# lmwdhr/ViT-CNN

Hardware: AMD Instinct MI355X
Metric: training patches/sec, 9×9 HSI(144)+LiDAR patch, batch 64, 1/2/4/8 GPU (higher is better)
Workload: dtype fp32; 1 GPU; ViT-CNN (Multimodality_Mamba) train step, Houston2013 shape 144+1 bands, 9x9, 16 classes; global_batch=64, per_gpu_batch=64, parallelism=dp1, launch=hipGraph (whole step)

## Files before the change

include/vitcnn.h:

```cpp
#ifndef VITCNN_H
#define VITCNN_H

#include <stddef.h>
#include <hip/hip_runtime_api.h>

#ifdef __cplusplus
#define VC_API extern "C" __attribute__((visibility("default")))
#else
#define VC_API __attribute__((visibility("default")))
#endif

VC_API int vc_gemm(int transA, int transB, int M, int N, int K, float alpha,
                   const float* A, long lda, long strideA, const float* B, long ldb, long strideB,
                   float beta, float* C, long ldc, long strideC, int batch,
                   const float* bias, const float* addend, long add_ld, int add_mod, int flags,
                   float* bias_grad, float* ws, long ws_floats, hipStream_t stream);
VC_API int vc_gemm_ex(int transA, int transB, int M, int N, int K, float alpha, const float* A, long lda,
                      long strideA, const float* B, long ldb, long strideB, float beta, float* C, long ldc,
                      long strideC, int batch, const float* bias, const float* addend, long add_ld, int add_mod,
                      int flags, float* bias_grad, float* ws, long ws_floats, unsigned int* tile_counters,
                      int n_counters, hipStream_t stream);

VC_API int vc_gemm_tune(int bm, int bn, int nsplit, int pf, int combine);

// ... 92 lines not shown
                           float* col, float* ws, long ws_floats, hipStream_t stream);
VC_API int vc_col2im3x3(int B, int H, int W, int C, const float* dcol, float* dx, hipStream_t stream);

VC_API int vc_nonlocal_attn_pool_fwd(int B, int S, int P, int Ci, int Hs, const float* theta, const float* pg,
                                     long ldpg, float* pooled, unsigned char* arg, float* att, float* o,
                                     hipStream_t stream);
VC_API int vc_nonlocal_attn_pool_bwd(int B, int S, int P, int Ci, int Hs, const float* theta, const float* pooled,
                                     const float* att, const float* dout, const unsigned char* arg, float* dtheta,
                                     float* dpooled, float* dpg, hipStream_t stream);
VC_API int vc_maxpool2_fwd(int B, int H, int W, int C, const float* x, long ldx, float* y, unsigned char* arg,
                           hipStream_t stream);
VC_API int vc_maxpool2_bwd(int B, int H, int W, int C, const float* dy, const unsigned char* arg, float* dx,
                           long lddx, hipStream_t stream);

VC_API int vc_mamba_dirconv_fwd(int B, int L, int D, int ndir, const int* order, const float* xz,
                                const float* conv_w, const float* conv_b, float* u, hipStream_t stream);
VC_API int vc_mamba_scan_ckpt_floats(int B, int L, int D, int ndir);
VC_API int vc_mamba_scan_fwd(int B, int L, int D, int R, int ndir, const float* u, const float* xdbl,
                             const int* order, const float* dt_w, const float* dt_b, const float* A_log,
                             const float* Dskip, float* yp, float* ckpt, hipStream_t stream);
VC_API int vc_mamba_combine_fwd(int B, int L, int D, int ndir, const int* inv_order, const float* gate_logits,
                                const float* yp, const float* xz, float* ypsum, float* ysum, hipStream_t stream);
VC_API int vc_mamba_gate_bwd(int B, int L, int D, const float* xz, const float* ypsum, const float* dysum,
                             float* dyp, float* dxz, hipStream_t stream);
VC_API int vc_mamba_scan_bwd(int B, int L, int D, int R, int ndir, const float* u, const float* xdbl,
                             const int* order, const float* dt_w, const float* dt_b, const float* A_log,
                             const float* Dskip, const float* gate_logits, const float* yp, const float* dyp,
                             const float* ckpt, float* du, float* ddt_lin, float* dxdbl, float* dA_log,
                             float* dDskip, float* dgate_logits, float* ws, long ws_floats, hipStream_t stream);
VC_API int vc_mamba_scan_bwd_params(int B, int D, int ndir, const float* gate_logits, const float* ws,
                                    float* dA_log, float* dDskip, float* dgate_logits, float* scratch,
                                    long scratch_floats, hipStream_t stream);
VC_API int vc_mamba_dirconv_bwd(int B, int L, int D, int ndir, const int* order, const int* inv_order,
                                const float* xz, const float* conv_w, const float* conv_b, float* du, float* dxz,
                                float* dconv_w, float* dconv_b, float* ws, long ws_floats, hipStream_t stream);
VC_API int vc_mamba_scan_fwd_fused(int B, int L, int D, int R, int ndir, const float* xz, const int* order,
                                   const float* conv_w, const float* conv_b, const float* x_proj_w,
                                   const float* dt_w, const float* dt_b, const float* A_log, const float* Dskip,
                                   float* u, float* xdbl, float* yp, float* ckpt, hipStream_t stream);
VC_API int vc_mamba_scan_bwd_fused(int B, int L, int D, int R, int ndir, const float* u, const float* xdbl,
                                   const int* order, const float* xz, const float* conv_w, const float* conv_b,
                                   const float* x_proj_w, const float* dt_w, const float* dt_b, const float* A_log,
                                   const float* Dskip, const float* gate_logits, const float* yp, const float* dyp,
                                   const float* ckpt, float* dpre, float* ddt_lin, float* dxdbl, float* conv_part,
                                   float* dA_log, float* dDskip, float* dgate_logits, float* ws, long ws_floats,
                                   hipStream_t stream);
VC_API int vc_mamba_dirconv_bwd_gather(int B, int L, int D, int ndir, const int* inv_order, const float* conv_w,
                                       const float* dpre, float* dxz, hipStream_t stream);
VC_API int vc_mamba_conv_params(int B, int D, int ndir, const float* conv_part, float* dconv_w, float* dconv_b,
                                hipStream_t stream);
VC_API int vc_mamba_bwd_params(int B, int D, int ndir, const float* gate_logits, const float* ws, const float* conv_part,
                               float* dA_log, float* dDskip, float* dgate_logits, float* dconv_w, float* dconv_b,
                               hipStream_t stream);

VC_API int vc_rowchain_front(int rows, int K0, int E, int N2, const float* x, const float* w_embed, const float* pos,
                             int L, float* t, const float* ln_w, const float* ln_b, float eps, float* xn, float* mean,
                             float* rstd, const float* w_proj, float* out, hipStream_t stream);
VC_API int vc_rowchain_back(int B, int L, int D, int ndir, const int* inv_order, const float* gate_logits,
                            const float* yp, const float* xz, float* ypsum, float* ysum, int E, const float* w_out,
                            const float* residual, float* t2, const float* ln_w, const float* ln_b, float eps,
                            float* g, float* mean, float* rstd, int N2, const float* w_proj, const float* b_proj,
                            float* out, hipStream_t stream);

VC_API int vc_rowchain_back_bwd(int rows, int Cout, int E, int D, const float* dcd, const float* w_cd, const float* t2,
                                const float* mean, const float* rstd, const float* ln_w, float* dt, float* ln_part,
                                const float* w_out, const float* xz, const float* ypsum, float* dyp, float* dxz,
                                hipStream_t stream);
VC_API int vc_rowchain_front_bwd(int rows, int K0, int E, int Cin, const float* dxz, const float* w_in, const float* t,
                                 const float* mean, const float* rstd, const float* ln_w, const float* res, float* dtt,
                                 float* ln_part, const float* w_embed, float* dx, float beta, const float* dx_add,
                                 hipStream_t stream);
VC_API int vc_rowchain_ln_params(int rows, int E, const float* ln_part, float* dw, float* db, float beta,
                                 hipStream_t stream);
VC_API int vc_rowchain_ln_part_floats(int rows, int E);

VC_API int vc_tl_ws_floats(int B, int HW, int S);
VC_API int vc_tl_check(int HW, int C, int S);
VC_API int vc_tl_pixel_stats(long M, int C, const float* x, long ldx, float* mx, int* amx, float* avg, double* ws,
                             hipStream_t stream);
VC_API int vc_tl_fwd(int train, int B, int HW, int C, int S, const float* x, long ldx, const float* mx,
                     const float* avg, const float* params, float* bn_buffers, float eps, float momentum,
                     const double* ws, double* stats, float* a, float* Z, hipStream_t stream);
VC_API int vc_tl_bwd(int train, int B, int HW, int C, int S, const float* x, long ldx, const float* mx,
                     const float* avg, const int* amx, const float* params, const double* stats, const float* a,
                     const float* dZ, double* ws, float* dx, long lddx, float* dparams, hipStream_t stream);
VC_API int vc_tl_relu_mask(int B, int HW, int S, const float* mx, const float* avg, const float* params,
                           const double* stats, unsigned char* mask, hipStream_t stream);

VC_API int vc_nonlocal_attn_fwd(int B, int S, int P, int Ci, const float* theta, const float* pooled, float* att,
                                float* o, hipStream_t stream);
VC_API int vc_nonlocal_attn_bwd(int B, int S, int P, int Ci, const float* theta, const float* pooled,
                                const float* att, const float* dout, float* dtheta, float* dpooled,
                                hipStream_t stream);

VC_API int vc_cat2_fwd(long M, int C1, int C2, const float* x1, long ld1, const float* x2, long ld2, int exchange,
                       float* out, hipStream_t stream);
VC_API int vc_cat2_bwd(long M, int C1, int C2, const float* dout, int exchange, float* dx1, long ld1, float beta1,
                       float* dx2, long ld2, float beta2, hipStream_t stream);
VC_API int vc_glf_combine_fwd(long M, int C, const float* w_pre, const float* bn_mean, const float* bn_invstd,
                              const float* bn_w, const float* bn_b, const float* fc, const float* fl, float* out,
                              hipStream_t stream);
VC_API int vc_bn_glf_combine(long M, int C, const float* w_pre, float eps, float momentum, float* save_mean,
                             float* save_invstd, float* run_mean, float* run_var, const float* bn_w, const float* bn_b,
                             const float* fc, const float* fl, float* out, float* ws, long ws_floats,
                             hipStream_t stream);
VC_API int vc_add2_2d(long M, int C, const float* a, long lda, const float* b, long ldb, float* out, long ldo,
// ... 170 lines not shown
```

vit-cnn_amd/csrc/mamba.hip:

```cpp
#include "common.h"

namespace {

constexpr int NST = 16;

constexpr int DC_T = 8;
__global__ void dirconv_fwd_run(int total, FastDiv fD, FastDiv fC, FastDiv fB, int L, const int* __restrict__ order,
                                const float* __restrict__ xz, const float* __restrict__ cw,
                                const float* __restrict__ cb, float* __restrict__ u) {
  const int idx = blockIdx.x * blockDim.x + threadIdx.x;
  if (idx >= total) return;
  const int D = fD.div;
  int d, c, b;
  const int sc = fdivmod(idx, fD, d);
  const int sq = fdivmod(sc, fC, c);
  const int k = fdivmod(sq, fB, b);
  const int* ord = order + k * L;
  const float* xb = xz + (long)b * L * (2 * D) + d;
  const float w0 = cw[d * 4], w1 = cw[d * 4 + 1], w2 = cw[d * 4 + 2], w3 = cw[d * 4 + 3], bias = cb[d];
  const int t0 = c * DC_T;
  float x[DC_T + 3];
#pragma unroll
  for (int i = 0; i < DC_T + 3; ++i) {
    const int tau = t0 - 3 + i;
// ... 749 lines not shown
  const int b = fdivmod(bl, fL, l);
  float mx = logits[0];
  for (int i = 1; i < ndir; ++i) mx = fmaxf(mx, logits[i]);
  float den = 0.f;
  for (int i = 0; i < ndir; ++i) den += __expf(logits[i] - mx);
  const float rden = 1.f / den;
  float acc = 0.f;
  for (int k0 = 0; k0 < ndir; k0 += MAXK) {
    int tk[MAXK];
#pragma unroll
    for (int kk = 0; kk < MAXK; ++kk) tk[kk] = k0 + kk < ndir ? inv[(k0 + kk) * L + l] : 0;
    float yv[MAXK];
#pragma unroll
    for (int kk = 0; kk < MAXK; ++kk)
      yv[kk] = k0 + kk < ndir ? y[((long)((k0 + kk) * B + b) * L + tk[kk]) * D + d] : 0.f;
#pragma unroll
    for (int kk = 0; kk < MAXK; ++kk)
      if (k0 + kk < ndir) {
        const float gk = __expf(logits[k0 + kk] - mx) * rden;
        acc += gk * yv[kk];
      }
  }
  ypsum[idx] = acc;
  out[idx] = acc * silu_f(xz[(long)bl * 2 * D + D + d]);
}

__device__ __forceinline__ void gate_grad_body(int ndir, int per_dir, const float* __restrict__ logits,
                                               const float* __restrict__ part, float* __restrict__ dlogits,
                                               float* dg, float* gg) {
  const int lane = threadIdx.x & 63, wave = threadIdx.x >> 6;
  for (int kk = wave; kk < ndir; kk += 4) {
    float s = 0.f;
    for (int i = lane; i < per_dir; i += 64) s += part[(long)kk * per_dir + i];
    s = wave_sum(s);
    if (lane == 0) {
      dg[kk] = s;
      gg[kk] = gate_softmax(logits, ndir, kk);
    }
  }
  __syncthreads();
  if (threadIdx.x < ndir) {
    float dot = 0.f;
    for (int i = 0; i < ndir; ++i) dot += gg[i] * dg[i];
    dlogits[threadIdx.x] = gg[threadIdx.x] * (dg[threadIdx.x] - dot);
  }
}

__global__ __launch_bounds__(256) void gate_grad(int ndir, int per_dir, const float* __restrict__ logits,
                                                 const float* __restrict__ part, float* __restrict__ dlogits) {
  __shared__ float dg[64], gg[64];
  gate_grad_body(ndir, per_dir, logits, part, dlogits, dg, gg);
}

__global__ __launch_bounds__(256) void mamba_params(int nseq, int D, int ndir, int ncb, const float* __restrict__ logits,
                                                    const float* __restrict__ pa, const float* __restrict__ pd,
                                                    const float* __restrict__ pg, const float* __restrict__ cp,
                                                    float* __restrict__ dA, float* __restrict__ dDs,
                                                    float* __restrict__ dgl, float* __restrict__ dcw,
                                                    float* __restrict__ dcb) {
  __shared__ float sh[16][17];
  __shared__ float dg[64], gg[64];
  if ((int)blockIdx.x == ncb) {
    gate_grad_body(ndir, nseq / ndir, logits, pg, dgl, dg, gg);
    return;
  }
  const int cl = threadIdx.x & 15, pl = threadIdx.x >> 4;
  const int c = blockIdx.x * 16 + cl;
  const float* src = nullptr;
  long stride = 0;
  float* dst = nullptr;
  int cc = 0;
  if (c < NST * D) src = pa, stride = (long)NST * D, dst = dA, cc = c;
  else if (c < (NST + 1) * D) src = pd, stride = D, dst = dDs, cc = c - NST * D;
  else if (c < (NST + 5) * D) src = cp, stride = 5L * D, dst = dcw, cc = c - (NST + 1) * D;
  else if (c < (NST + 6) * D) src = cp + 4L * D, stride = 5L * D, dst = dcb, cc = c - (NST + 5) * D;
  float s = 0.f;
  if (src) {
#pragma unroll 4
    for (int p = pl; p < nseq; p += 16) s += src[(long)p * stride + cc];
  }
  sh[pl][cl] = s;
  __syncthreads();
  if (pl == 0 && src) {
    float v = 0.f;
#pragma unroll
    for (int i = 0; i < 16; ++i) v += sh[i][cl];
    dst[cc] = v;
  }
}


template <int MAXK>
__global__ void dirconv_bwd_gather(int total, FastDiv fD, FastDiv fL, int B, int ndir, const int* __restrict__ inv,
                                   const float* __restrict__ cw, const float* __restrict__ dpre,
                                   float* __restrict__ dxz) {
  const int idx = blockIdx.x * blockDim.x + threadIdx.x;
  if (idx >= total) return;
  const int D = fD.div, L = fL.div;
  int d, l;
  const int bl = fdivmod(idx, fD, d);
  const int b = fdivmod(bl, fL, l);
  float w[4];
#pragma unroll
  for (int j = 0; j < 4; ++j) w[j] = cw[d * 4 + j];
  float acc = 0.f;
  for (int k0 = 0; k0 < ndir; k0 += MAXK) {
    int tk[MAXK];
#pragma unroll
    for (int kk = 0; kk < MAXK; ++kk) tk[kk] = k0 + kk < ndir ? inv[(k0 + kk) * L + l] : L;
    float v[MAXK][4];
#pragma unroll
    for (int kk = 0; kk < MAXK; ++kk) {
      const float* base = dpre + (long)((k0 + kk) * B + b) * L * D + d;
#pragma unroll
      for (int j = 0; j < 4; ++j) {
        const int t = tk[kk] + 3 - j;
        v[kk][j] = t < L ? base[(long)t * D] : 0.f;
      }
    }
#pragma unroll
    for (int kk = 0; kk < MAXK; ++kk)
#pragma unroll
      for (int j = 0; j < 4; ++j) acc = fmaf(w[j], v[kk][j], acc);
  }
  dxz[(long)bl * 2 * D + d] = acc;
}

__global__ __launch_bounds__(256) void dirconv_bwd_wgrad(int D, int L, FastDiv fC, FastDiv fB,
                                                         const int* __restrict__ order, const float* __restrict__ xz,
                                                         const float* __restrict__ cw, const float* __restrict__ cb,
                                                         float* __restrict__ du, int items, int items_per,
                                                         float* __restrict__ part) {
  __shared__ float sh[5][16][17];
  const int dlc = threadIdx.x & 15, rl = threadIdx.x >> 4;
  const int d = blockIdx.x * 16 + dlc;
  const int i0 = blockIdx.y * items_per, i1 = min(items, i0 + items_per);
  float acc[5] = {0.f, 0.f, 0.f, 0.f, 0.f};
  if (d < D) {
    const float w0 = cw[d * 4], w1 = cw[d * 4 + 1], w2 = cw[d * 4 + 2], w3 = cw[d * 4 + 3], bias = cb[d];
    for (int it = i0 + rl; it < i1; it += 16) {
// ... 220 lines not shown
                                   float* u, float* xdbl, float* y, float* ckpt, hipStream_t stream) {
  VC_REQUIRE(B > 0 && L > 0 && D > 0 && D <= 128 && R > 0 && R <= 64 && ndir > 0);
  VC_REQUIRE(xz && order && conv_w && conv_b && x_proj_w && u && xdbl && scan_fusable(D, R));
  const dim3 grid(ndir * B), block(vc_cdiv(D, 16) * 64);
  VC_REQUIRE(block.x <= 512);
  const size_t sm = sizeof(float) * (seq_lds_floats(L, R, block.x / 4) + L);
  VC_REQUIRE(sm <= 160 * 1024);
  VC_REQUIRE_I32((long)ndir * B * L * (R + 2 * NST));
  VC_REQUIRE_I32((long)B * L * 2 * D);
  const ScanArgs a{B, L, D, R, u, xdbl, order, dt_w, dt_b, A_log, Dskip};
  const FusedFwd f{xz, conv_w, conv_b, x_proj_w, u, xdbl};
  if (R == 9) hipLaunchKernelGGL((scan_fwd<9, true>), grid, block, sm, stream, a, y, ckpt, f);
  else if (R == 16) hipLaunchKernelGGL((scan_fwd<16, true>), grid, block, sm, stream, a, y, ckpt, f);
  else hipLaunchKernelGGL((scan_fwd<0, true>), grid, block, sm, stream, a, y, ckpt, f);
  VC_CHECK_LAUNCH();
  return VC_OK;
}

VC_API int vc_mamba_dirconv_bwd_gather(int B, int L, int D, int ndir, const int* inv_order, const float* conv_w,
                                       const float* dpre, float* dxz, hipStream_t stream) {
  VC_REQUIRE(B > 0 && L > 0 && D > 0 && ndir > 0);
  VC_REQUIRE_I32((long)ndir * B * L * D);
  const long tot2 = (long)B * L * D;
  if (ndir <= 10)
    hipLaunchKernelGGL(dirconv_bwd_gather<10>, dim3(vc_cdiv(tot2, 256)), dim3(256), 0, stream, (int)tot2,
                       make_fastdiv(D), make_fastdiv(L), B, ndir, inv_order, conv_w, dpre, dxz);
  else
    hipLaunchKernelGGL(dirconv_bwd_gather<4>, dim3(vc_cdiv(tot2, 256)), dim3(256), 0, stream, (int)tot2,
                       make_fastdiv(D), make_fastdiv(L), B, ndir, inv_order, conv_w, dpre, dxz);
  VC_CHECK_LAUNCH();
  return VC_OK;
}

VC_API int vc_mamba_conv_params(int B, int D, int ndir, const float* conv_part, float* dconv_w, float* dconv_b,
                                hipStream_t stream) {
  VC_REQUIRE(B > 0 && D > 0 && ndir > 0 && conv_part && dconv_w && dconv_b);
  const int nseq = ndir * B;
  if (dconv_b == dconv_w + 4L * D) return launch_sum_rows(nseq, 5 * D, conv_part, 5L * D, 0L, dconv_w, 0.f, stream);
  const int rc = launch_sum_rows(nseq, 4 * D, conv_part, 5L * D, 0L, dconv_w, 0.f, stream);
  if (rc) return rc;
  return launch_sum_rows(nseq, D, conv_part, 5L * D, 4L * D, dconv_b, 0.f, stream);
}

VC_API int vc_mamba_bwd_params(int B, int D, int ndir, const float* gate_logits, const float* ws, const float* conv_part,
                               float* dA_log, float* dDskip, float* dgate_logits, float* dconv_w, float* dconv_b,
                               hipStream_t stream) {
  VC_REQUIRE(B > 0 && D > 0 && ndir > 0 && ndir <= 64 && gate_logits && ws && conv_part && dA_log && dDskip &&
             dgate_logits && dconv_w && dconv_b);
  const int nseq = ndir * B;
  const float* p_a = ws;
  const float* p_d = p_a + (long)nseq * D * NST;
  const float* p_g = p_d + (long)nseq * D;
  const int ncb = vc_cdiv((NST + 6) * D, 16);
  hipLaunchKernelGGL(mamba_params, dim3(ncb + 1), dim3(256), 0, stream, nseq, D, ndir, ncb, gate_logits, p_a, p_d,
                     p_g, conv_part, dA_log, dDskip, dgate_logits, dconv_w, dconv_b);
  VC_CHECK_LAUNCH();
  return VC_OK;
}

VC_API int vc_mamba_scan_bwd_params(int B, int D, int ndir, const float* gate_logits, const float* ws,
                                    float* dA_log, float* dDskip, float* dgate_logits, float* scratch,
                                    long scratch_floats, hipStream_t stream) {
  VC_REQUIRE(B > 0 && D > 0 && ndir > 0 && ws);
  const int nseq = ndir * B;
  const float* p_a = ws;
  const float* p_d = p_a + (long)nseq * D * NST;
  const float* p_g = p_d + (long)nseq * D;
  return scan_param_reduce(B, D, ndir, gate_logits, p_a, p_d, p_g, dA_log, dDskip, dgate_logits, scratch,
                           scratch_floats, stream);
}


VC_API int vc_mamba_dirconv_bwd(int B, int L, int D, int ndir, const int* order, const int* inv_order, const float* xz,
                                const float* conv_w, const float* conv_b, float* du, float* dxz,
                                float* dconv_w, float* dconv_b, float* ws, long ws_floats, hipStream_t stream) {
  VC_REQUIRE(B > 0 && L > 0 && D > 0 && ndir > 0);
  const long rows = (long)ndir * B * L;
  VC_REQUIRE_I32(rows * D);
  const int nch = vc_cdiv(L, DC_T);
  const long items = (long)ndir * B * nch;
  int items_per = std::max<long>(16, (items + 255) / 256);
  while ((long)vc_cdiv(items, items_per) * D * 5 > ws_floats) items_per *= 2;
  const int P = vc_cdiv(items, items_per);
  hipLaunchKernelGGL(dirconv_bwd_wgrad, dim3(vc_cdiv(D, 16), P), dim3(256), 0, stream, D, L, make_fastdiv(nch),
                     make_fastdiv(B), order, xz, conv_w, conv_b, du, (int)items, items_per, ws);
  VC_CHECK_LAUNCH();
  const long tot2 = (long)B * L * D;
  if (ndir <= 10)
    hipLaunchKernelGGL(dirconv_bwd_gather<10>, dim3(vc_cdiv(tot2, 256)), dim3(256), 0, stream, (int)tot2,
                       make_fastdiv(D), make_fastdiv(L), B, ndir, inv_order, conv_w, du, dxz);
  else
    hipLaunchKernelGGL(dirconv_bwd_gather<4>, dim3(vc_cdiv(tot2, 256)), dim3(256), 0, stream, (int)tot2,
                       make_fastdiv(D), make_fastdiv(L), B, ndir, inv_order, conv_w, du, dxz);
  VC_CHECK_LAUNCH();
  if (dconv_b == dconv_w + 4L * D) return launch_sum_rows(P, 5 * D, ws, 5L * D, 0L, dconv_w, 0.f, stream);
  int rc = launch_sum_rows(P, 4 * D, ws, 5L * D, 0L, dconv_w, 0.f, stream);
  if (rc) return rc;
  rc = launch_sum_rows(P, D, ws, 5L * D, 4L * D, dconv_b, 0.f, stream);
  if (rc) return rc;
  return VC_OK;
}
```

vit-cnn_amd/vitcnn_amd/model.py:

```python
from __future__ import annotations

import contextlib
import ctypes
import math
import sys
import weakref
from typing import Dict

import torch
import torch.nn as nn

from ._lib import lib
from .flat import install_grad_views
from .layers import ConvBnReluParams, FusionParams, GlobalLocalParams
from .scan_orders import scan_orders

F32 = 4
LN_EPS = 1e-6
BN_EPS = 1e-5
BN_MOM = 0.1
NDIR = 10
N_SIDE = 3
_ONE_PARAM_REDUCE = True
WGRAD_LANE = 2
WGRAD1_LANE = 3
_IMPLICIT_CONV = False
_DEFER_WGRAD = True
_DEFER_WGRAD1 = False
SIDE_SCRATCH = 1 << 23
PARAM_ALIGN = 4
ALIGN_MIN = 64
GEMM_GROUP_BYTES = 16384
GEMM_MASK = 64
_GLOBAL_FIRST = False
_GEMM_BNSTATS = True
_PG_LANE2 = False
N_COUNTERS = 1 << 16

_SCAN_FUSED = True
_ROW_CHAIN = True
_GLF_FUSED = True
_TAP_DGRAD = False
_LANES = True
_LANES_BWD = True
_TRACER = None
_GROUP = True
_BF16_EXACT: set = set()
_BF16_MIN_K = 0
_GEMM_SITES = None
_LANE_MAP = []
_CH_LANE = 1
_CH_ORDERED = True
_BN_RELU_AFFINE = True
_BN_TICKETS = False

UNUSED_PREFIXES = ("hsi1.global_view.tokenlearner.", "hsi1.global_view.ln3.",
                   "hsi2.global_view.tokenlearner.", "hsi2.global_view.ln3.")


PRECISIONS = ("fp32", "bf16")
GEMM_BF16 = 2


def _check_precision(p):
    if p not in PRECISIONS:
        raise ValueError(f"precision must be one of {PRECISIONS}, got {p!r}")
    return p


class _Workspace:

    def __init__(self, device):
        self.device = device
        self.t: Dict[str, torch.Tensor] = {}
        self.generation = 0

# ... 998 lines not shown
                if dX:
                    self.mm_nn(rows, Cin, Cout, dCF, Cout, self.P[pfx + ".channel_feature.weight"], Cin, dX, Cin,
                               beta=1.0)
            e_ch = (self.mark(), e_loc) if side else (self.mark(),)
            self.flush_wgrads1()
        Zg, dZg = f(pfx + ".global_feature.Z", M * Cout), f(pfx + ".dZg", M * Cout)
        self.ln_bwd(pfx + ".ln3", pfx + ".Fg", dFg, Zg, M, Cout, dZg, 0.0, defer=True)
        CD, dCD = f(pfx + ".CD", rows * Cout), f(pfx + ".dCD", rows * Cout)
        self.token_learner_bwd(pfx + ".global_feature", CD, L_, Cout, S, dZg, dCD)
        Gm, dG = f(pfx + ".G", rows * E), f(pfx + ".dG", rows * E)
        T2, dT = f(pfx + ".T2", rows * E), f(pfx + ".dT", rows * E)
        YS, dYS = f(pfx + ".YS", rows * D), f(pfx + ".dYS", rows * D)
        U, XD, XZ = f(pfx + ".U", NDIR * rows * D), f(pfx + ".XD", NDIR * rows * XW), f(pfx + ".XZ", rows * 2 * D)
        Y, YP = f(pfx + ".Y", NDIR * rows * D), f(pfx + ".YP", rows * D)
        dU, dDTL = f(pfx + ".dU", NDIR * rows * D), f(pfx + ".dDTL", NDIR * rows * D)
        dXD, dXZ, dYP = f(pfx + ".dXD", NDIR * rows * XW), f(pfx + ".dXZ", rows * 2 * D), f(pfx + ".dYP", rows * D)
        if self._chain_back_bwd_ok(blk):
            part = f(pfx + ".ln1part", self.L.vc_rowchain_ln_part_floats(rows, E))
            self.L.vc_rowchain_back_bwd(rows, Cout, E, D, dCD, P[pfx + ".change_dim.weight"], T2, f(pfx + ".G.m", rows),
                                        f(pfx + ".G.r", rows), P[gv + ".ln1.weight"], dT, part,
                                        P[mx + ".out_proj.weight"], XZ, YP, dYP, dXZ, self.s)
            self.defer_wgrad(True, Cout, E, rows, dCD, Cout, Gm, E, G[pfx + ".change_dim.weight"], E,
                             G[pfx + ".change_dim.bias"])
            self._ln_params(gv + ".ln1", rows, E, part)
            self.defer_wgrad(True, E, D, rows, dT, E, YS, D, G[mx + ".out_proj.weight"], D)
        else:
            self.linear_bwd(pfx + ".change_dim.weight", pfx + ".change_dim.bias", dCD, rows, Cout, E, Gm, E, dG, 0.0,
                            defer=True)
            self.ln_bwd(gv + ".ln1", pfx + ".G", dG, T2, rows, E, dT, 0.0, defer=True)
            self.linear_bwd(mx + ".out_proj.weight", None, dT, rows, E, D, YS, D, dYS, 0.0, defer=True)
            self.L.vc_mamba_gate_bwd(B, L_, D, XZ, YP, dYS, dYP, dXZ, self.s)
        self.flush_wgrads()
        CKPb = f(pfx + ".CKP", self.L.vc_mamba_scan_ckpt_floats(B, L_, D, NDIR))
        if self.scan_fused:
            self._scan_bwd_fused(pfx, gv, mx, B, L_, D, R, XW, order, inv, CKPb)
            return self._block_bwd_tail(blk, pfx, gv, mx, B, L_, E, Cin, rows, X, dX, dT, e_ch)
        if self._deferring(True):
            nseq = NDIR * B
            spn = nseq * D * 16 + nseq * D + nseq
            sp = f(pfx + ".scanpart", spn)
            self.L.vc_mamba_scan_bwd(B, L_, D, R, NDIR, U, XD, order, P[mx + ".dt_proj.weight"],
                                     P[mx + ".dt_proj.bias"], P[mx + ".A_log"], P[mx + ".D"], P[gv + ".weights"], Y,
                                     dYP, CKPb, dU, dDTL, dXD, None, None, None, sp, spn, self.s)
            gl, ga, gd, gg = P[gv + ".weights"], G[mx + ".A_log"], G[mx + ".D"], G[gv + ".weights"]
            self.pending_wgrads.append(
                lambda: self.L.vc_mamba_scan_bwd_params(B, D, NDIR, gl, sp, ga, gd, gg, self.scr_p, self.scr_n,
                                                        self.s))
        else:
            self.L.vc_mamba_scan_bwd(B, L_, D, R, NDIR, U, XD, order, P[mx + ".dt_proj.weight"],
                                     P[mx + ".dt_proj.bias"], P[mx + ".A_log"], P[mx + ".D"], P[gv + ".weights"], Y,
                                     dYP, CKPb, dU, dDTL, dXD, G[mx + ".A_log"], G[mx + ".D"], G[gv + ".weights"],
                                     self.scr_p, self.scr_n, self.s)
        nr = NDIR * rows
        self.defer_wgrad(True, D, R, nr, dDTL, D, XD, XW, G[mx + ".dt_proj.weight"], R, G[mx + ".dt_proj.bias"])
        self.mm_nn(nr, R, D, dDTL, D, P[mx + ".dt_proj.weight"], R, dXD, XW)
        self.linear_bwd(mx + ".x_proj.weight", None, dXD, nr, XW, D, U, D, dU, 1.0, defer=True)
        self.L.vc_mamba_dirconv_bwd(B, L_, D, NDIR, order, inv, XZ, P[mx + ".conv1d.weight"], P[mx + ".conv1d.bias"],
                                    dU, dXZ, G[mx + ".conv1d.weight"], G[mx + ".conv1d.bias"], self.scr_p,
                                    self.scr_n, self.s)
        self._block_bwd_tail(blk, pfx, gv, mx, B, L_, E, Cin, rows, X, dX, dT, e_ch)

    def _scan_bwd_fused(self, pfx, gv, mx, B, L_, D, R, XW, order, inv, CKPb):
        P, G, f = self.P, self.G, self.ws.f
        rows = B * L_
        nr, nseq = NDIR * rows, NDIR * B
        U, XD, XZ = f(pfx + ".U", nr * D), f(pfx + ".XD", nr * XW), f(pfx + ".XZ", rows * 2 * D)
        Y, dYP = f(pfx + ".Y", nr * D), f(pfx + ".dYP", rows * D)
        dU, dDTL, dXD, dXZ = f(pfx + ".dU", nr * D), f(pfx + ".dDTL", nr * D), f(pfx + ".dXD", nr * XW), f(
            pfx + ".dXZ", rows * 2 * D)
        CP = f(pfx + ".convpart", nseq * 5 * D)
        defer = self._deferring(True)
        spn = nseq * D * 16 + nseq * D + nseq
        sp = f(pfx + ".scanpart", spn)
        gl, ga, gd, gg = P[gv + ".weights"], G[mx + ".A_log"], G[mx + ".D"], G[gv + ".weights"]
        self.L.vc_mamba_scan_bwd_fused(B, L_, D, R, NDIR, U, XD, order, XZ, P[mx + ".conv1d.weight"],
                                       P[mx + ".conv1d.bias"], P[mx + ".x_proj.weight"], P[mx + ".dt_proj.weight"],
                                       P[mx + ".dt_proj.bias"], P[mx + ".A_log"], P[mx + ".D"], gl, Y, dYP, CKPb, dU,
                                       dDTL, dXD, CP, None, None, None, sp, spn, self.s)
        cw, cb = G[mx + ".conv1d.weight"], G[mx + ".conv1d.bias"]
        if _ONE_PARAM_REDUCE:
            params = lambda: self.L.vc_mamba_bwd_params(B, D, NDIR, gl, sp, CP, ga, gd, gg, cw, cb, self.s)
        else:
            def params():
                self.L.vc_mamba_scan_bwd_params(B, D, NDIR, gl, sp, ga, gd, gg, self.scr_p, self.scr_n, self.s)
                self.L.vc_mamba_conv_params(B, D, NDIR, CP, cw, cb, self.s)
        if defer:
            self.pending_wgrads.append(params)
        else:
            params()
        self.L.vc_mamba_dirconv_bwd_gather(B, L_, D, NDIR, inv, P[mx + ".conv1d.weight"], dU, dXZ, self.s)
        self.defer_wgrad(True, D, R, nr, dDTL, D, XD, XW, G[mx + ".dt_proj.weight"], R, G[mx + ".dt_proj.bias"])
        self.defer_wgrad(True, XW, D, nr, dXD, XW, U, D, G[mx + ".x_proj.weight"], D)

    def _chain_ok(self, blk):
        E = blk.embed
        return (self.row_chain and blk.cin <= 256 and blk.cin % 4 == 0 and E <= 256 and E % 4 == 0
                and (E // 2) % 4 == 0 and blk.cout <= 256)

    def _chain_back_bwd_ok(self, blk):
        return self._chain_ok(blk) and blk.cout % 4 == 0

    def _ln_params(self, pfx, rows, E, part):
        gw, gb = self.G[pfx + ".weight"], self.G[pfx + ".bias"]
        fn = lambda: self.L.vc_rowchain_ln_params(rows, E, part, gw, gb, 0.0, self.s)
        if self._deferring(True):
            self.pending_wgrads.append(fn)
        else:
            fn()

    def _block_bwd_tail(self, blk, pfx, gv, mx, B, L_, E, Cin, rows, X, dX, dT, e_ch):
        ws, P, G, f = self.ws, self.P, self.G, self.ws.f
        D = E // 2
        dXZ = f(pfx + ".dXZ", rows * 2 * D)
        Xn, dXn = f(pfx + ".Xn", rows * E), f(pfx + ".dXn", rows * E)
        T, dTt = f(pfx + ".T", rows * E), f(pfx + ".dTt", rows * E)
        if self._chain_ok(blk):
            self.defer_wgrad(True, 2 * D, E, rows, dXZ, 2 * D, Xn, E, G[mx + ".in_proj.weight"], E)
            self.flush_wgrads()
            if dX:
                self.wait(*e_ch)
            part = f(pfx + ".prepart", self.L.vc_rowchain_ln_part_floats(rows, E))
            self.L.vc_rowchain_front_bwd(rows, 2 * D, E, Cin, dXZ, P[mx + ".in_proj.weight"], T, f(pfx + ".Xn.m", rows),
                                         f(pfx + ".Xn.r", rows), P[gv + ".pre_norm.weight"], dT, dTt, part,
                                         P[gv + ".patch_embed.projection.weight"], dX or None, 1.0, None, self.s)
            self._ln_params(gv + ".pre_norm", rows, E, part)
        else:
            self.linear_bwd(mx + ".in_proj.weight", None, dXZ, rows, 2 * D, E, Xn, E, dXn, 0.0, defer=True)
            self.flush_wgrads()
            self.ln_bwd(gv + ".pre_norm", pfx + ".Xn", dXn, T, rows, E, dTt, 0.0, res=dT, defer=True)
            if dX:
                self.wait(*e_ch)
                self.mm_nn(rows, Cin, E, dTt, E, P[gv + ".patch_embed.projection.weight"], Cin, dX, Cin, beta=1.0)
        e = self.mark()
        with self.lane(WGRAD_LANE if _DEFER_WGRAD else 0, e):
            self.colsum(B, L_ * E, dTt, L_ * E, G[gv + ".pos_embed"])
            self.mm_tn(E, Cin, rows, dTt, E, X, Cin, G[gv + ".patch_embed.projection.weight"], Cin)
            if self.lanes_on and _DEFER_WGRAD:
                self.wgrad_tail = self.mark()

    def bucket_ready(self, hook, name, *side_events):
        if hook is None:
            return
        assert self.cur == 0
        hook(name, [self.mark()] + list(side_events))

# ... 41 lines not shown
```

Before: 39060 patches/s.

## Fuse dt_proj and x_proj weight gradients into one MFMA kernel with partial reduction

Adds a dedicated proj_wgrad kernel that computes the dt_proj weight/bias gradients and the x_proj weight gradient in a single pass over the rows. It uses double-buffered buffer loads into LDS and MFMA 16x16x4 accumulation, with each of 256 blocks writing a partial record. The partials are then reduced in a combined params kernel that also absorbs the existing scan/conv parameter reduction, replacing two separate deferred wgrad GEMMs and one launch. This trades generic GEMM calls for a fixed-grid specialised kernel that only applies when D<=128 and R<=16, and it adds workspace for the partial records.

```diff
diff --git a/include/vitcnn.h b/include/vitcnn.h
--- a/include/vitcnn.h
+++ b/include/vitcnn.h
@@ -168,6 +168,14 @@
 VC_API int vc_mamba_bwd_params(int B, int D, int ndir, const float* gate_logits, const float* ws, const float* conv_part,
                                float* dA_log, float* dDskip, float* dgate_logits, float* dconv_w, float* dconv_b,
                                hipStream_t stream);
+VC_API int vc_mamba_proj_wgrad_check(int D, int R);
+VC_API int vc_mamba_proj_wgrad_ws_floats(long rows, int D, int R);
+VC_API int vc_mamba_proj_wgrad(long rows, int D, int R, const float* ddt_lin, const float* xdbl, const float* dxdbl,
+                               const float* u, float* part, long part_floats, hipStream_t stream);
+VC_API int vc_mamba_bwd_params_proj(int B, int D, int R, int ndir, const float* gate_logits, const float* ws,
+                                    const float* conv_part, const float* proj_part, int nrec, float* dA_log,
+                                    float* dDskip, float* dgate_logits, float* dconv_w, float* dconv_b, float* ddt_w,
+                                    float* ddt_b, float* dx_proj_w, hipStream_t stream);
 
 VC_API int vc_rowchain_front(int rows, int K0, int E, int N2, const float* x, const float* w_embed, const float* pos,
                              int L, float* t, const float* ln_w, const float* ln_b, float eps, float* xn, float* mean,
diff --git a/vit-cnn_amd/csrc/mamba.hip b/vit-cnn_amd/csrc/mamba.hip
--- a/vit-cnn_amd/csrc/mamba.hip
+++ b/vit-cnn_amd/csrc/mamba.hip
@@ -825,20 +825,29 @@
   gate_grad_body(ndir, per_dir, logits, part, dlogits, dg, gg);
 }
 
-__global__ __launch_bounds__(256) void mamba_params(int nseq, int D, int ndir, int ncb, const float* __restrict__ logits,
-                                                    const float* __restrict__ pa, const float* __restrict__ pd,
-                                                    const float* __restrict__ pg, const float* __restrict__ cp,
-                                                    float* __restrict__ dA, float* __restrict__ dDs,
-                                                    float* __restrict__ dgl, float* __restrict__ dcw,
-                                                    float* __restrict__ dcb) {
+struct ParamsArgs {
+  int nseq, D, ndir, ncb;
+  const float *logits, *pa, *pd, *pg, *cp;
+  float *dA, *dDs, *dgl, *dcw, *dcb;
+};
+
+__device__ __forceinline__ void mamba_params_block(int bid, const ParamsArgs& a) {
+  const int nseq = a.nseq, D = a.D, ndir = a.ndir, ncb = a.ncb;
+  const float* __restrict__ pa = a.pa;
+  const float* __restrict__ pd = a.pd;
+  const float* __restrict__ cp = a.cp;
+  float* __restrict__ dA = a.dA;
+  float* __restrict__ dDs = a.dDs;
+  float* __restrict__ dcw = a.dcw;
+  float* __restrict__ dcb = a.dcb;
   __shared__ float sh[16][17];
   __shared__ float dg[64], gg[64];
-  if ((int)blockIdx.x == ncb) {
-    gate_grad_body(ndir, nseq / ndir, logits, pg, dgl, dg, gg);
+  if (bid == ncb) {
+    gate_grad_body(ndir, nseq / ndir, a.logits, a.pg, a.dgl, dg, gg);
     return;
   }
   const int cl = threadIdx.x & 15, pl = threadIdx.x >> 4;
-  const int c = blockIdx.x * 16 + cl;
+  const int c = bid * 16 + cl;
   const float* src = nullptr;
   long stride = 0;
   float* dst = nullptr;
@@ -859,6 +868,197 @@
 #pragma unroll
     for (int i = 0; i < 16; ++i) v += sh[i][cl];
     dst[cc] = v;
+  }
+}
+
+__global__ __launch_bounds__(256) void mamba_params(ParamsArgs a) { mamba_params_block((int)blockIdx.x, a); }
+
+constexpr int PW_NB = 256;
+constexpr int PW_KC = 32;
+constexpr int PW_ND = 2;
+constexpr int PW_NX = 6;
+
+static int pw_pitch(int D) { return (D + 47) / 64 * 64 + 16; }
+
+struct ProjStage {
+  float4 dd[PW_ND], uu[PW_ND], xd[PW_NX], dx[PW_NX];
+};
+
+struct ProjSrc {
+  __amdgpu_buffer_rsrc_t dd, uu, xd, dx;
+};
+constexpr unsigned PW_OOB = 0x80000000u;
+
+__device__ __forceinline__ float4 buf_ld4(__amdgpu_buffer_rsrc_t r, unsigned off) {
+  return __builtin_bit_cast(float4, __builtin_amdgcn_raw_buffer_load_b128(r, off, 0, 0));
+}
+
+__device__ __forceinline__ void pw_load(ProjStage& st, const ProjSrc& src, int cr, int D, int XW, const FastDiv& fD4) {
+  const int tid = threadIdx.x, nt = blockDim.x;
+#pragma unroll
+  for (int i = 0; i < PW_ND; ++i) {
+    int c4;
+    const int row = fdivmod(tid + i * nt, fD4, c4);
+    const unsigned off = row < PW_KC ? (unsigned)((cr + row) * D + 4 * c4) * 4u : PW_OOB;
+    st.dd[i] = buf_ld4(src.dd, off);
+    st.uu[i] = buf_ld4(src.uu, off);
+  }
+#pragma unroll
+  for (int i = 0; i < PW_NX; ++i) {
+    const int q = tid + i * nt;
+    const unsigned off = q < PW_KC * XW / 4 ? (unsigned)(cr * XW + 4 * q) * 4u : PW_OOB;
+    st.xd[i] = buf_ld4(src.xd, off);
+    st.dx[i] = buf_ld4(src.dx, off);
+  }
+}
+
+__device__ __forceinline__ void pw_tail(long c0, long r1, int XW, const float* __restrict__ xd,
+                                        const float* __restrict__ dxd, float* sXD, float* sDX) {
+  const long end = r1 * XW, t0 = end & ~3L, base = c0 * XW;
+  if (t0 == end || t0 < base || t0 >= base + (long)PW_KC * XW) return;
+  if ((long)threadIdx.x < end - t0) {
+    sXD[t0 - base + threadIdx.x] = xd[t0 + threadIdx.x];
+    sDX[t0 - base + threadIdx.x] = dxd[t0 + threadIdx.x];
+  }
+  __syncthreads();
+}
+
+__device__ __forceinline__ void pw_store(const ProjStage& st, int D, int Dp, int XW, const FastDiv& fD4, float* sDD,
+                                         float* sU, float* sXD, float* sDX) {
+  const int tid = threadIdx.x, nt = blockDim.x;
+#pragma unroll
+  for (int i = 0; i < PW_ND; ++i) {
+    int c4;
+    const int row = fdivmod(tid + i * nt, fD4, c4);
+    if (row < PW_KC) {
+      *reinterpret_cast<float4*>(sDD + row * Dp + 4 * c4) = st.dd[i];
+      *reinterpret_cast<float4*>(sU + row * Dp + 4 * c4) = st.uu[i];
+    }
+  }
+#pragma unroll
+  for (int i = 0; i < PW_NX; ++i) {
+    const int q = tid + i * nt;
+    if (q < PW_KC * XW / 4) {
+      *reinterpret_cast<float4*>(sXD + 4 * q) = st.xd[i];
+      *reinterpret_cast<float4*>(sDX + 4 * q) = st.dx[i];
+    }
+  }
+}
+
+template <bool FULL, bool R16>
+__device__ __forceinline__ void pw_mma(int nk, int Dp, int XW, int R, int wave, int g, int l16, const float* sDD,
+                                       const float* sU, const float* sXD, const float* sDX, f32x4 (&acc1)[2],
+                                       f32x4 (&acc2)[3]) {
+  const float one0 = l16 == 0 ? 1.f : 0.f;
+#pragma unroll 1
+  for (int kb = 0; kb < PW_KC / 4; kb += 4) {
+#pragma unroll
+    for (int ks = kb; ks < kb + 4; ++ks) {
+      if (!FULL && ks >= nk) return;
+      const int kr = 4 * ks + g;
+      const float a1 = sDD[kr * Dp + 16 * wave + l16];
+      const float bu = sU[kr * Dp + 16 * wave + l16];
+      const float xv = sXD[kr * XW + l16];
+      const float b1 = l16 < R ? xv : (l16 == R ? 1.f : 0.f);
+      acc1[0] = __builtin_amdgcn_mfma_f32_16x16x4f32(a1, b1, acc1[0], 0, 0, 0);
+      if (R16) acc1[1] = __builtin_amdgcn_mfma_f32_16x16x4f32(a1, one0, acc1[1], 0, 0, 0);
+#pragma unroll
+      for (int xt = 0; xt < 3; ++xt)
+        acc2[xt] = __builtin_amdgcn_mfma_f32_16x16x4f32(sDX[kr * XW + 16 * xt + l16], bu, acc2[xt], 0, 0, 0);
+    }
+  }
+}
+
+template <bool R16>
+__global__ __launch_bounds__(512) void proj_wgrad(long rows, int slice, int D, int R, int Dp, FastDiv fD4, int phases,
+                                                  const float* __restrict__ ddtl, const float* __restrict__ xd,
+                                                  const float* __restrict__ dxd, const float* __restrict__ u,
+                                                  float* __restrict__ part) {
+  extern __shared__ __align__(16) float pw_sm[];
+  const int XW = R + 2 * NST;
+  const int nxw = PW_KC * XW + 16;
+  float* sDD = pw_sm;
+  float* sU = sDD + PW_KC * Dp;
+  float* sXD = sU + PW_KC * Dp;
+  float* sDX = sXD + nxw;
+  const int tid = threadIdx.x, lane = tid & 63, wave = tid >> 6, g = lane >> 4, l16 = lane & 15;
+  const long r0 = (long)blockIdx.x * slice, r1 = r0 + slice < rows ? r0 + slice : rows;
+  const int nrow = r1 > r0 ? (int)(r1 - r0) : 0;
+  const int nchunk = (nrow + PW_KC - 1) / PW_KC;
+  const unsigned dbytes = phases & 1 ? (unsigned)(nrow * D) * 4u : 0u;
+  const unsigned xbytes = nrow && (phases & 1) ? (unsigned)(((r1 * XW) & ~3L) - r0 * XW) * 4u : 0u;
+  const ProjSrc src{buf_rsrc(ddtl + r0 * D, dbytes), buf_rsrc(u + r0 * D, dbytes), buf_rsrc(xd + r0 * XW, xbytes),
+                    buf_rsrc(dxd + r0 * XW, xbytes)};
+  ProjStage st[2];
+  pw_load(st[0], src, 0, D, XW, fD4);
+  pw_load(st[1], src, PW_KC, D, XW, fD4);
+  for (int i = tid; i < 2 * PW_KC * Dp + 2 * nxw; i += blockDim.x) pw_sm[i] = 0.f;
+  __syncthreads();
+  f32x4 acc1[2] = {}, acc2[3] = {};
+  for (int c = 0; c < nchunk; c += 2) {
+#pragma unroll
+    for (int h = 0; h < 2; ++h) {
+      const int cr = (c + h) * PW_KC;
+      pw_store(st[h], D, Dp, XW, fD4, sDD, sU, sXD, sDX);
+      __syncthreads();
+      pw_load(st[h], src, cr + 2 * PW_KC, D, XW, fD4);
+      pw_tail(r0 + cr, r1, XW, xd, dxd, sXD, sDX);
+      if (!(phases & 2)) {
+      } else if (nrow - cr >= PW_KC)
+        pw_mma<true, R16>(PW_KC / 4, Dp, XW, R, wave, g, l16, sDD, sU, sXD, sDX, acc1, acc2);
+      else
+        pw_mma<false, R16>((nrow - cr + 3) / 4, Dp, XW, R, wave, g, l16, sDD, sU, sXD, sDX, acc1, acc2);
+      __syncthreads();
+    }
+  }
+  float* rec = part + (long)blockIdx.x * ((long)D * R + D + (long)XW * D);
+  float* rec_b = rec + D * R;
+  float* rec_x = rec_b + D;
+#pragma unroll
+  for (int r = 0; r < 4; ++r) {
+    const int d = 16 * wave + 4 * g + r;
+    if (d < D) {
+      if (l16 < R) rec[d * R + l16] = acc1[0][r];
+      else if (l16 == R) rec_b[d] = acc1[0][r];
+      if (R16 && l16 == 0) rec_b[d] = acc1[1][r];
+    }
+  }
+  const int dc = 16 * wave + l16;
+#pragma unroll
+  for (int xt = 0; xt < 3; ++xt)
+#pragma unroll
+    for (int r = 0; r < 4; ++r) {
+      const int x = 16 * xt + 4 * g + r;
+      if (x < XW && dc < D) rec_x[x * D + dc] = acc2[xt][r];
+    }
+}
+
+__global__ __launch_bounds__(256) void mamba_params_proj(ParamsArgs a, int first, int nrec, int DR, int recn,
+                                                         const float* __restrict__ pp, float* __restrict__ ddt_w,
+                                                         float* __restrict__ ddt_b, float* __restrict__ dxw) {
+  if ((int)blockIdx.x < first) {
+    mamba_params_block((int)blockIdx.x, a);
+    return;
+  }
+  __shared__ float sh[16][17];
+  const int cl = threadIdx.x & 15, pl = threadIdx.x >> 4;
+  const int c = ((int)blockIdx.x - first) * 16 + cl;
+  float* dst = nullptr;
+  if (c < DR) dst = ddt_w + c;
+  else if (c < DR + a.D) dst = ddt_b + (c - DR);
+  else if (c < recn) dst = dxw + (c - DR - a.D);
+  float s = 0.f;
+  if (dst) {
+#pragma unroll 4
+    for (int p = pl; p < nrec; p += 16) s += pp[(long)p * recn + c];
+  }
+  sh[pl][cl] = s;
+  __syncthreads();
+  if (pl == 0 && dst) {
+    float v = 0.f;
+#pragma unroll
+    for (int i = 0; i < 16; ++i) v += sh[i][cl];
+    *dst = v;
   }
 }
 
@@ -1185,8 +1385,63 @@
   const float* p_d = p_a + (long)nseq * D * NST;
   const float* p_g = p_d + (long)nseq * D;
   const int ncb = vc_cdiv((NST + 6) * D, 16);
-  hipLaunchKernelGGL(mamba_params, dim3(ncb + 1), dim3(256), 0, stream, nseq, D, ndir, ncb, gate_logits, p_a, p_d,
-                     p_g, conv_part, dA_log, dDskip, dgate_logits, dconv_w, dconv_b);
+  const ParamsArgs a{nseq, D, ndir, ncb, gate_logits, p_a, p_d, p_g, conv_part, dA_log, dDskip, dgate_logits, dconv_w,
+                     dconv_b};
+  hipLaunchKernelGGL(mamba_params, dim3(ncb + 1), dim3(256), 0, stream, a);
+  VC_CHECK_LAUNCH();
+  return VC_OK;
+}
+
+static bool proj_wgrad_ok(int D, int R) { return D > 0 && D <= 128 && D % 4 == 0 && R >= 1 && R <= 16; }
+static long proj_rec_floats(int D, int R) { return (long)D * R + D + (long)(R + 2 * NST) * D; }
+
+VC_API int vc_mamba_proj_wgrad_check(int D, int R) { return proj_wgrad_ok(D, R) ? VC_OK : VC_EINVAL; }
+
+VC_API int vc_mamba_proj_wgrad_ws_floats(long rows, int D, int R) {
+  if (rows <= 0 || !proj_wgrad_ok(D, R)) return -1;
+  return (int)(PW_NB * proj_rec_floats(D, R));
+}
+
+VC_API int vc_mamba_proj_wgrad(long rows, int D, int R, const float* ddt_lin, const float* xdbl, const float* dxdbl,
+                               const float* u, float* part, long part_floats, hipStream_t stream) {
+  VC_REQUIRE(rows > 0 && proj_wgrad_ok(D, R) && ddt_lin && xdbl && dxdbl && u && part);
+  VC_REQUIRE_I32(rows);
+  VC_REQUIRE(part_floats >= PW_NB * proj_rec_floats(D, R));
+  VC_REQUIRE(((uintptr_t)ddt_lin | (uintptr_t)xdbl | (uintptr_t)dxdbl | (uintptr_t)u) % 16 == 0);
+  const int XW = R + 2 * NST, Dp = pw_pitch(D);
+  const int slice = vc_cdiv(vc_cdiv(rows, PW_NB), 4) * 4;
+  VC_REQUIRE_I32(((long)slice + 3 * PW_KC) * (D > XW ? D : XW) * 4);
+  const size_t sm = sizeof(float) * (2 * PW_KC * Dp + 2 * (PW_KC * XW + 16));
+  const dim3 grid(PW_NB), block(vc_cdiv(D, 16) * 64);
+  const int phases = (int)vc_knob("VITCNN_PROJ_PHASES", 3);
+  if (R == 16)
+    hipLaunchKernelGGL(proj_wgrad<true>, grid, block, sm, stream, rows, slice, D, R, Dp, make_fastdiv(D / 4), phases,
+                       ddt_lin, xdbl, dxdbl, u, part);
+  else
+    hipLaunchKernelGGL(proj_wgrad<false>, grid, block, sm, stream, rows, slice, D, R, Dp, make_fastdiv(D / 4), phases,
+                       ddt_lin, xdbl, dxdbl, u, part);
+  VC_CHECK_LAUNCH();
+  return VC_OK;
+}
+
+VC_API int vc_mamba_bwd_params_proj(int B, int D, int R, int ndir, const float* gate_logits, const float* ws,
+                                    const float* conv_part, const float* proj_part, int nrec, float* dA_log,
+                                    float* dDskip, float* dgate_logits, float* dconv_w, float* dconv_b, float* ddt_w,
+                                    float* ddt_b, float* dx_proj_w, hipStream_t stream) {
+  VC_REQUIRE(B > 0 && ndir > 0 && ndir <= 64 && proj_wgrad_ok(D, R) && proj_part && nrec > 0 && ddt_w && ddt_b &&
+             dx_proj_w);
+  VC_REQUIRE(!ws || (gate_logits && conv_part && dA_log && dDskip && dgate_logits && dconv_w && dconv_b));
+  const int nseq = ndir * B;
+  const float* p_a = ws;
+  const float* p_d = ws ? p_a + (long)nseq * D * NST : nullptr;
+  const float* p_g = ws ? p_d + (long)nseq * D : nullptr;
+  const int ncb = vc_cdiv((NST + 6) * D, 16);
+  const int first = ws ? ncb + 1 : 0;
+  const int recn = (int)proj_rec_floats(D, R);
+  const ParamsArgs a{nseq, D, ndir, ncb, gate_logits, p_a, p_d, p_g, conv_part, dA_log, dDskip, dgate_logits, dconv_w,
+                     dconv_b};
+  hipLaunchKernelGGL(mamba_params_proj, dim3(first + vc_cdiv(recn, 16)), dim3(256), 0, stream, a, first, nrec, D * R,
+                     recn, proj_part, ddt_w, ddt_b, dx_proj_w);
   VC_CHECK_LAUNCH();
   return VC_OK;
 }
diff --git a/vit-cnn_amd/vitcnn_amd/model.py b/vit-cnn_amd/vitcnn_amd/model.py
--- a/vit-cnn_amd/vitcnn_amd/model.py
+++ b/vit-cnn_amd/vitcnn_amd/model.py
@@ -22,6 +22,7 @@
 NDIR = 10
 N_SIDE = 3
 _ONE_PARAM_REDUCE = True
+_PROJ_WGRAD = True
 WGRAD_LANE = 2
 WGRAD1_LANE = 3
 _IMPLICIT_CONV = False
@@ -1126,9 +1127,15 @@
                                      dYP, CKPb, dU, dDTL, dXD, G[mx + ".A_log"], G[mx + ".D"], G[gv + ".weights"],
                                      self.scr_p, self.scr_n, self.s)
         nr = NDIR * rows
-        self.defer_wgrad(True, D, R, nr, dDTL, D, XD, XW, G[mx + ".dt_proj.weight"], R, G[mx + ".dt_proj.bias"])
+        proj = self._proj_wgrad_ok(D, R)
+        if not proj:
+            self.defer_wgrad(True, D, R, nr, dDTL, D, XD, XW, G[mx + ".dt_proj.weight"], R, G[mx + ".dt_proj.bias"])
         self.mm_nn(nr, R, D, dDTL, D, P[mx + ".dt_proj.weight"], R, dXD, XW)
-        self.linear_bwd(mx + ".x_proj.weight", None, dXD, nr, XW, D, U, D, dU, 1.0, defer=True)
+        if proj:
+            self.mm_nn(nr, D, XW, dXD, XW, P[mx + ".x_proj.weight"], D, dU, D, beta=1.0)
+            self._proj_wgrad(pfx, mx, B, nr, D, R, dDTL, XD, dXD, U)
+        else:
+            self.linear_bwd(mx + ".x_proj.weight", None, dXD, nr, XW, D, U, D, dU, 1.0, defer=True)
         self.L.vc_mamba_dirconv_bwd(B, L_, D, NDIR, order, inv, XZ, P[mx + ".conv1d.weight"], P[mx + ".conv1d.bias"],
                                     dU, dXZ, G[mx + ".conv1d.weight"], G[mx + ".conv1d.bias"], self.scr_p,
                                     self.scr_n, self.s)
@@ -1152,19 +1159,46 @@
                                        P[mx + ".dt_proj.bias"], P[mx + ".A_log"], P[mx + ".D"], gl, Y, dYP, CKPb, dU,
                                        dDTL, dXD, CP, None, None, None, sp, spn, self.s)
         cw, cb = G[mx + ".conv1d.weight"], G[mx + ".conv1d.bias"]
-        if _ONE_PARAM_REDUCE:
+        proj = self._proj_wgrad_ok(D, R)
+        if proj and _ONE_PARAM_REDUCE:
+            params = None
+        elif _ONE_PARAM_REDUCE:
             params = lambda: self.L.vc_mamba_bwd_params(B, D, NDIR, gl, sp, CP, ga, gd, gg, cw, cb, self.s)
         else:
             def params():
                 self.L.vc_mamba_scan_bwd_params(B, D, NDIR, gl, sp, ga, gd, gg, self.scr_p, self.scr_n, self.s)
                 self.L.vc_mamba_conv_params(B, D, NDIR, CP, cw, cb, self.s)
-        if defer:
+        if params and defer:
             self.pending_wgrads.append(params)
-        else:
+        elif params:
             params()
         self.L.vc_mamba_dirconv_bwd_gather(B, L_, D, NDIR, inv, P[mx + ".conv1d.weight"], dU, dXZ, self.s)
+        if proj:
+            self._proj_wgrad(pfx, mx, B, nr, D, R, dDTL, XD, dXD, U,
+                             (gl, sp, CP, ga, gd, gg, cw, cb) if params is None else None)
+            return
         self.defer_wgrad(True, D, R, nr, dDTL, D, XD, XW, G[mx + ".dt_proj.weight"], R, G[mx + ".dt_proj.bias"])
         self.defer_wgrad(True, XW, D, nr, dXD, XW, U, D, G[mx + ".x_proj.weight"], D)
+
+    def _proj_wgrad_ok(self, D, R):
+        return _PROJ_WGRAD and self.L.raw["vc_mamba_proj_wgrad_check"](D, R) == 0
+
+    def _proj_wgrad(self, pfx, mx, B, nr, D, R, dDTL, XD, dXD, U, scan=None):
+        G = self.G
+        ppn = self.L.vc_mamba_proj_wgrad_ws_floats(nr, D, R)
+        pp = self.ws.f(pfx + ".projpart", ppn)
+        nrec = ppn // (D * R + D + (R + 32) * D)
+        gw, gb, gx = G[mx + ".dt_proj.weight"], G[mx + ".dt_proj.bias"], G[mx + ".x_proj.weight"]
+        scan = scan or (None,) * 8
+
+        def fn():
+            self.L.vc_mamba_proj_wgrad(nr, D, R, dDTL, XD, dXD, U, pp, ppn, self.s)
+            self.L.vc_mamba_bwd_params_proj(B, D, R, NDIR, scan[0], scan[1], scan[2], pp, nrec, *scan[3:], gw, gb, gx,
+                                            self.s)
+        if self._deferring(True):
+            self.pending_wgrads.append(fn)
+        else:
+            fn()
 
     def _chain_ok(self, blk):
         E = blk.embed
```

Result: no change. 39220 patches/s, median of 5 (+0.4%).
